# PythonerJOJO/GenPose2

Hardware: AMD Instinct MI355X
Metric: pose candidates/sec (B objs x K cands x T denoise steps) (higher is better)
Workload: dtype f32 (pose_encoder.2 / head-1 GEMMs: f16x3 -- three f16 planes per fp32 operand, six MFMA products, products to 2^-33, fp32 accumulation; encoder SA levels 1-3: split-f16, per-level error vs float64 within exact fp32 MFMA's: tests/test_gpu_precision.py); 1 GPU; config4: B=256 objects/GPU, N=1024 pts, K=50 candidates, T=500 PC steps, ScoreNet+EnergyNet+ranking/aggregation (encoder + sampler per step); global_batch=256, seq_len=500, parallelism=dp1 (object shards), encoder_pipelined=False, energy_encoder=beside the score encoder

## Files before the change

### genpose2_amd/csrc/gp_encoder.hip

```cpp
#include <algorithm>

#include "gp_common.h"
#include "gp_fps.h"
#include "gp_head.h"

int gp_launch_fps_chain(const float* xyz, int b, int nlev, const int* n, const int* m, int* const* idx,
                        float* const* nxyz, hipStream_t st);
int gp_launch_ball_query2(int b, int n, int m, float ra, float rb, int nsa, int nsb, const float* new_xyz,
                          const float* xyz, int* idxa, int* idxb, hipStream_t st);

struct SAArgs {
    int n_prev, c_prev, m, ns, cols;
    const float* xyz_prev;
    const float* feat_prev;
    const float* cent;
    const int* nbr;
    int nlayers;
    const float* w[3];
    const float* bias[3];
    int kg[3];
    int nt[3];
    float* out;
    int c_out_total, out_off;
    int buf1_off;
// ... 501 lines not shown
    f32x4 acc[2 * NC][CT];
#pragma unroll
    for (int t = 0; t < 2 * NC; ++t)
#pragma unroll
        for (int ct = 0; ct < CT; ++ct) acc[t][ct] = f32x4{0.f, 0.f, 0.f, 0.f};
    stream_hk_step<KC1, 0, D, 2 * NC, CT, D>(W, T, X, lane, voff, ring, acc);
    __syncthreads();
    SPLIT_MARK(a, 6);
    stream_hk_step<KC1, D, KC1 + D, 2 * NC, CT, D>(W, T, X, lane, voff, ring, acc);
    const int span = a.ns >> 4;
#pragma unroll
    for (int t = 0; t < 2 * NC; ++t) {
        const f32x4 bias = ld4(a.bias[1] + 16 * T[t] + 4 * q);
        f32x4 v[CT];
#pragma unroll
        for (int ct = 0; ct < CT; ++ct) v[ct] = relu4(acc[t][ct] * exp2i(e1[ct] - 14 - a.ew[1]) + bias);
#pragma unroll
        for (int ct = 0; ct < CT; ++ct) {
            if (span == 2) {
                if (ct & 1) continue;
                v[ct] = vmax4(v[ct], v[ct + 1]);
            }
            const float r = row16_max_scatter4(v[ct], n);
            const int mi = (col0 + ct * 16) / a.ns;
            if ((n & 3) == 0 && mi < a.m) a.out[((size_t)b * a.m + mi) * a.c_out_total + a.out_off + 16 * T[t] + 4 * q + (n >> 2)] = r;
        }
    }
}

template <int CT, int D, int KC0, int OC1, int OC2>
__device__ __forceinline__ void sa_split_body(const SplitArgs& a, char* smem) {
    constexpr int C = 16 * CT, KX = KC0 > OC1 ? KC0 : OC1;
    f16x8* X = reinterpret_cast<f16x8*>(smem);
    float* P = reinterpret_cast<float*>(smem + (size_t)KX * CT * 2048);
    float* pm = P + CT * KC0 * 32;
    int* e0s = reinterpret_cast<int*>(pm + SPLIT_WV * C);
    const int tid = threadIdx.x, lane = tid & 63;
    const int wid = __builtin_amdgcn_readfirstlane(tid >> 6);
    const int b = blockIdx.y, col0 = blockIdx.x * C;
    SPLIT_MARK(a, 0);
    constexpr bool EARLY = KC0 >= 8;
    f32x4 gq[KC0][2];
    const int pnb = wid < CT ? split_gather0_pre(a, b, col0, wid, lane) : 0;
    split_centroid_term<CT, KC0>(a, P, b, col0, tid);
    if (EARLY && wid < CT) split_gather0_load<KC0>(a, b, pnb, lane, gq);
    if constexpr (EARLY) {
        asm volatile("s_waitcnt lgkmcnt(0)\n\ts_barrier" ::: "memory");
    } else {
        __syncthreads();
    }
    SPLIT_MARK(a, 1);
    int e1[CT];
    constexpr int NC1_HI = (OC1 + SPLIT_WV - 1) / SPLIT_WV;
    const int nc1 = wid < OC1 % SPLIT_WV || OC1 % SPLIT_WV == 0 ? NC1_HI : NC1_HI - 1;
    if (nc1 == NC1_HI)
        split_layer1<CT, KC0, NC1_HI, D>(a, X, e0s, pm, reinterpret_cast<const f32x4*>(P), b, col0, wid, lane, OC1, e1, gq, EARLY, pnb);
    else
        split_layer1<CT, KC0, (NC1_HI > 0 ? NC1_HI - 1 : 0), D>(a, X, e0s, pm, reinterpret_cast<const f32x4*>(P), b, col0, wid, lane, OC1, e1, gq, EARLY, pnb);
    static_assert(OC2 % SPLIT_WV == 0, "layer-2 chunks spread evenly over the waves");
    split_layer2<CT, OC1, OC2 / SPLIT_WV, D>(a, X, e1, b, col0, wid, lane, OC2);
    SPLIT_MARK(a, 7);
}

template <int CT, int D, int KC0, int OC1A, int OC2A, int OC1B, int OC2B, int MINB = 1>
__global__ __launch_bounds__(SPLIT_WV * 64) __attribute__((amdgpu_waves_per_eu(2 * MINB))) void sa_split_kernel(SplitArgs a0, SplitArgs a1) {
    extern __shared__ __attribute__((aligned(16))) char smem[];
    if (blockIdx.z == 0) {
        if ((int)blockIdx.x * 16 * CT < a0.cols) sa_split_body<CT, D, KC0, OC1A, OC2A>(a0, smem);
    } else {
        if ((int)blockIdx.x * 16 * CT < a1.cols) sa_split_body<CT, D, KC0, OC1B, OC2B>(a1, smem);
    }
}

#ifndef SPLIT_CT2
#define SPLIT_CT2 4
#endif
#ifndef SPLIT_CT3
#define SPLIT_CT3 6
#endif
#ifndef SPLIT_D2
#define SPLIT_D2 2
#endif
#ifndef SPLIT_D3
#define SPLIT_D3 2
#endif

template <int CT, int KC0, int OC1>
static size_t sa_split_lds() {
    constexpr int KX = KC0 > OC1 ? KC0 : OC1;
    return (size_t)KX * CT * 2048 + sizeof(float) * CT * KC0 * 32 + sizeof(float) * SPLIT_WV * 16 * CT + sizeof(int) * 16 * CT;
}

struct NarrowArgs {
    const float* qin;
    int q_stride, q_off, n_prev;
    const float* w0;
    int kg0, gx;
    const float* w1;
    const float* b1;
    const float* w2;
    const float* b2;
    const int* nbr;
    const float* cent;
    int m, ns, nobj;
    float* out;
    int c_out_total, out_off;
    const float* w1h;
    const float* w2h;
    int ew1, ew2;
};

template <int SPAN, int KG>
struct NarrowGather {
    f32x4 q[SPAN][KG];
    float cx, cy, cz;
};

template <int SPAN>
__device__ __forceinline__ void narrow_nbr(const NarrowArgs& a, int task, int nn, int (&p)[SPAN]) {
#pragma unroll
    for (int ct = 0; ct < SPAN; ++ct) p[ct] = a.nbr[(size_t)task * a.ns + ct * 16 + nn];
}

template <int KG>
__device__ __forceinline__ const f32x4* narrow_centroid_term(const f32x4* sW0x, int q, float cx, float cy, float cz,
                                                             f32x4 (&cw)[KG]) {
#pragma clang fp contract(off)
#pragma unroll
    for (int g = 0; g < KG; ++g) {
        float r[4];
#pragma unroll
        for (int j = 0; j < 4; ++j) {
            const f32x4 wx = sW0x[16 * g + 4 * q + j];
            r[j] = (wx.x * cx + wx.y * cy) + wx.z * cz;
        }
        cw[g] = f32x4{r[0], r[1], r[2], r[3]};
    }
    return cw;
}

template <int SPAN, int KG>
__device__ __forceinline__ void narrow_fetch(const NarrowArgs& a, int task, const int (&p)[SPAN], int q,
                                             NarrowGather<SPAN, KG>& g) {
    const int b = task / a.m;
    const float* cc = a.cent + (size_t)task * 3;
    g.cx = ld1(cc);
    g.cy = ld1(cc + 1);
    g.cz = ld1(cc + 2);
#pragma unroll
    for (int ct = 0; ct < SPAN; ++ct) {
        const float* qrow = a.qin + ((size_t)b * a.n_prev + p[ct]) * a.q_stride + a.q_off + 4 * q;
#pragma unroll
        for (int g2 = 0; g2 < KG; ++g2) g.q[ct][g2] = ld4(qrow + 16 * g2);
    }
}

template <int KG1, int NT1, int NT2, int SPAN>
__device__ __forceinline__ void narrow_branch(const NarrowArgs& a, f32x4* lds) {
    constexpr int KG2 = NT1;
    constexpr int NA1 = NT1 * KG1 * 64, NA2 = NT2 * KG2 * 64;
    f32x4* sA1 = lds;
    f32x4* sA2 = sA1 + NA1;
    f32x4* sW0x = sA2 + NA2;
    float* sB1 = reinterpret_cast<float*>(sW0x + KG1 * 16);
    float* sB2 = sB1 + NT1 * 16;
    const int tid = threadIdx.x;
    for (int i = tid; i < NA1; i += SA_THREADS) sA1[i] = ld4(a.w1 + (size_t)i * 4);
    for (int i = tid; i < NA2; i += SA_THREADS) sA2[i] = ld4(a.w2 + (size_t)i * 4);
    for (int ch = tid; ch < KG1 * 16; ch += SA_THREADS)
        sW0x[ch] = ld4(a.w0 + ((size_t)((ch >> 4) * a.kg0 + a.gx) * 64 + (ch & 15)) * 4);
    for (int i = tid; i < NT1 * 16; i += SA_THREADS) sB1[i] = a.b1[i];
    for (int i = tid; i < NT2 * 16; i += SA_THREADS) sB2[i] = a.b2[i];
    __syncthreads();
    const int lane = tid & 63, q = lane >> 4, nn = lane & 15;
    const int nw = gridDim.x * (SA_THREADS / 64);
    const int total = a.nobj * a.m;
    int task = blockIdx.x * (SA_THREADS / 64) + (tid >> 6);
    if (task >= total) return;
    int pn[SPAN];
    NarrowGather<SPAN, KG1> cur, nxt;
    f32x4 cwv[KG1];
    narrow_nbr<SPAN>(a, task, nn, pn);
    narrow_fetch<SPAN, KG1>(a, task, pn, q, cur);
    if (task + nw < total) narrow_nbr<SPAN>(a, task + nw, nn, pn);
    for (; task < total; task += nw) {
        if (task + nw < total) {
            narrow_fetch<SPAN, KG1>(a, task + nw, pn, q, nxt);
            if (task + 2 * nw < total) narrow_nbr<SPAN>(a, task + 2 * nw, nn, pn);
        }
        const float cx = cur.cx, cy = cur.cy, cz = cur.cz;
        f32x4 rmax[NT2];
#pragma unroll
        for (int t = 0; t < NT2; ++t) rmax[t] = f32x4{NEG_BIG, NEG_BIG, NEG_BIG, NEG_BIG};
        const f32x4* cw = narrow_centroid_term<KG1>(sW0x, q, cx, cy, cz, cwv);
#pragma unroll
        for (int ct = 0; ct < SPAN; ++ct) {
            f32x4 bf[KG1];
#pragma unroll
            for (int g = 0; g < KG1; ++g) {
                float r[4];
#pragma unroll
                for (int j = 0; j < 4; ++j) r[j] = relu1(fsub(cur.q[ct][g][j], cw[g][j]));
                bf[g] = f32x4{r[0], r[1], r[2], r[3]};
            }
            f32x4 acc1[NT1];
#pragma unroll
            for (int t = 0; t < NT1; ++t) acc1[t] = f32x4{0.f, 0.f, 0.f, 0.f};
#pragma unroll
            for (int g = 0; g < KG1; ++g) {
                f32x4 af[NT1];
#pragma unroll
                for (int t = 0; t < NT1; ++t) af[t] = sA1[(t * KG1 + g) * 64 + lane];
#pragma unroll
                for (int j = 0; j < 4; ++j)
#pragma unroll
                    for (int t = 0; t < NT1; ++t) acc1[t] = mfma4(af[t][j], bf[g][j], acc1[t]);
                __builtin_amdgcn_sched_barrier(0);
            }
#pragma unroll
            for (int t = 0; t < NT1; ++t) acc1[t] = relu4(acc1[t] + ld4(&sB1[16 * t + 4 * q]));
            f32x4 acc2[NT2];
#pragma unroll
            for (int t = 0; t < NT2; ++t) acc2[t] = f32x4{0.f, 0.f, 0.f, 0.f};
#pragma unroll
            for (int g = 0; g < KG2; ++g) {
                f32x4 af[NT2];
#pragma unroll
                for (int t = 0; t < NT2; ++t) af[t] = sA2[(t * KG2 + g) * 64 + lane];
#pragma unroll
                for (int j = 0; j < 4; ++j)
#pragma unroll
                    for (int t = 0; t < NT2; ++t) acc2[t] = mfma4(af[t][j], acc1[g][j], acc2[t]);
                __builtin_amdgcn_sched_barrier(0);
            }
#pragma unroll
            for (int t = 0; t < NT2; ++t) rmax[t] = vmax4(rmax[t], acc2[t]);
            __builtin_amdgcn_sched_barrier(0);
        }
        float* o = a.out + (size_t)task * a.c_out_total + a.out_off + 4 * q;
#pragma unroll
        for (int t = 0; t < NT2; ++t) {
            const int j = nn >> 2;
            const float r = relu1(row16_max_scatter4(rmax[t], nn) + sB2[16 * t + 4 * q + j]);
            if ((nn & 3) == 0) o[16 * t + j] = r;
        }
        cur = nxt;
    }
}

template <int KC0, int NT1, int NT2, int SPAN>
__device__ __forceinline__ void narrow_branch_split(const NarrowArgs& a, f32x4* lds) {
    constexpr int KG1 = 2 * KC0, KC1 = NT1 / 2;
    static_assert(NT1 % 2 == 0, "layer-1 tiles pair into 32-deep chunks");
    constexpr int NA1 = NT1 * KC0 * 2 * 64, NA2 = NT2 * KC1 * 2 * 64;
    f16x8* sA1 = reinterpret_cast<f16x8*>(lds);
    f16x8* sA2 = sA1 + NA1;
    f32x4* sW0x = reinterpret_cast<f32x4*>(sA2 + NA2);
    float* sB1 = reinterpret_cast<float*>(sW0x + KG1 * 16);
    float* sB2 = sB1 + NT1 * 16;
    const int tid = threadIdx.x;
    for (int i = tid; i < NA1; i += SA_THREADS) sA1[i] = __builtin_bit_cast(f16x8, ld4(a.w1h + (size_t)i * 4));
    for (int i = tid; i < NA2; i += SA_THREADS) sA2[i] = __builtin_bit_cast(f16x8, ld4(a.w2h + (size_t)i * 4));
    for (int ch = tid; ch < KG1 * 16; ch += SA_THREADS)
        sW0x[ch] = ld4(a.w0 + ((size_t)((ch >> 4) * a.kg0 + a.gx) * 64 + (ch & 15)) * 4);
    for (int i = tid; i < NT1 * 16; i += SA_THREADS) sB1[i] = a.b1[i];
    for (int i = tid; i < NT2 * 16; i += SA_THREADS) sB2[i] = a.b2[i];
    __syncthreads();
    const int lane = tid & 63, q = lane >> 4, nn = lane & 15;
    const int nw = gridDim.x * (SA_THREADS / 64);
    const int total = a.nobj * a.m;
    int task = blockIdx.x * (SA_THREADS / 64) + (tid >> 6);
    if (task >= total) return;
    int pn[SPAN];
    NarrowGather<SPAN, KG1> cur, nxt;
    f32x4 cwv[KG1];
    narrow_nbr<SPAN>(a, task, nn, pn);
    narrow_fetch<SPAN, KG1>(a, task, pn, q, cur);
    if (task + nw < total) narrow_nbr<SPAN>(a, task + nw, nn, pn);
    for (; task < total; task += nw) {
        if (task + nw < total) {
            narrow_fetch<SPAN, KG1>(a, task + nw, pn, q, nxt);
            if (task + 2 * nw < total) narrow_nbr<SPAN>(a, task + 2 * nw, nn, pn);
        }
        const float cx = cur.cx, cy = cur.cy, cz = cur.cz;
        f32x4 rmax[NT2];
#pragma unroll
        for (int t = 0; t < NT2; ++t) rmax[t] = f32x4{NEG_BIG, NEG_BIG, NEG_BIG, NEG_BIG};
        const f32x4* cw = narrow_centroid_term<KG1>(sW0x, q, cx, cy, cz, cwv);
#pragma unroll
        for (int ct = 0; ct < SPAN; ++ct) {
            f32x4 bf[KG1];
            float mx = 0.f;
#pragma unroll
            for (int g = 0; g < KG1; ++g) {
                float r[4];
#pragma unroll
                for (int j = 0; j < 4; ++j) {
                    r[j] = relu1(fsub(cur.q[ct][g][j], cw[g][j]));
                    mx = fmax2(mx, r[j]);
                }
                bf[g] = f32x4{r[0], r[1], r[2], r[3]};
            }
            const int E0 = col_exponent(rows_max(mx));
            f16x8 h0[KC0], l0[KC0];
#pragma unroll
            for (int c = 0; c < KC0; ++c) split_pair(bf[2 * c], bf[2 * c + 1], exp2i(14 - E0), h0[c], l0[c]);
            f32x4 acc1[NT1];
#pragma unroll
            for (int t = 0; t < NT1; ++t) acc1[t] = f32x4{0.f, 0.f, 0.f, 0.f};
#pragma unroll
            for (int c = 0; c < KC0; ++c) {
#pragma unroll
                for (int t = 0; t < NT1; ++t) {
                    const f16x8 ah = sA1[((t * KC0 + c) * 2 + 0) * 64 + lane];
                    const f16x8 al = sA1[((t * KC0 + c) * 2 + 1) * 64 + lane];
                    acc1[t] = mfma_h(al, h0[c], acc1[t]);
                    acc1[t] = mfma_h(ah, l0[c], acc1[t]);
                    acc1[t] = mfma_h(ah, h0[c], acc1[t]);
                }
            }
            const float u0 = exp2i(E0 - 14 - a.ew1);
            float m1 = 0.f;
#pragma unroll
            for (int t = 0; t < NT1; ++t) {
                acc1[t] = relu4(acc1[t] * u0 + ld4(&sB1[16 * t + 4 * q]));
                m1 = fmax2(m1, max4(acc1[t]));
            }
            const int E1 = col_exponent(rows_max(m1));
            f16x8 h1[KC1], l1[KC1];
#pragma unroll
            for (int c = 0; c < KC1; ++c) split_pair(acc1[2 * c], acc1[2 * c + 1], exp2i(14 - E1), h1[c], l1[c]);
            f32x4 acc2[NT2];
#pragma unroll
            for (int t = 0; t < NT2; ++t) acc2[t] = f32x4{0.f, 0.f, 0.f, 0.f};
#pragma unroll
            for (int c = 0; c < KC1; ++c) {
#pragma unroll
                for (int t = 0; t < NT2; ++t) {
                    const f16x8 ah = sA2[((t * KC1 + c) * 2 + 0) * 64 + lane];
                    const f16x8 al = sA2[((t * KC1 + c) * 2 + 1) * 64 + lane];
                    acc2[t] = mfma_h(al, h1[c], acc2[t]);
                    acc2[t] = mfma_h(ah, l1[c], acc2[t]);
                    acc2[t] = mfma_h(ah, h1[c], acc2[t]);
                }
            }
            const float u1 = exp2i(E1 - 14 - a.ew2);
#pragma unroll
            for (int t = 0; t < NT2; ++t) rmax[t] = vmax4(rmax[t], acc2[t] * u1);
            __builtin_amdgcn_sched_barrier(0);
        }
        float* o = a.out + (size_t)task * a.c_out_total + a.out_off + 4 * q;
#pragma unroll
        for (int t = 0; t < NT2; ++t) {
            const int j = nn >> 2;
            const float r = relu1(row16_max_scatter4(rmax[t], nn) + sB2[16 * t + 4 * q + j]);
            if ((nn & 3) == 0) o[16 * t + j] = r;
        }
        cur = nxt;
    }
}

struct FpsSide {
    int nlev;
    int n[2], m[2], nb[2], jbits[2];
    const float* in;
    int* idx[2];
    float* nxyz[2];
    int nobj;
};

static size_t fps_side_lds(const FpsSide& f) {
    return f.nlev ? FPS_RED_BYTES + sizeof(float) * 3 * ((size_t)f.n[0] + f.m[0]) + sizeof(int) * (size_t)f.m[0] : 0;
}

__device__ __forceinline__ void fps_side(const FpsSide& f, char* smem) {
    const int b = blockIdx.x;
    if (b >= f.nobj) return;
    void* s_red = smem;
    float* cur = reinterpret_cast<float*>(smem + FPS_RED_BYTES);
    float* nxt = cur + 3 * f.n[0];
    int* s_idx = reinterpret_cast<int*>(nxt + 3 * f.m[0]);
    const float* src = f.in + (size_t)b * f.n[0] * 3;
    for (int i = threadIdx.x; i < 3 * f.n[0]; i += FPS_THREADS) cur[i] = src[i];
    __syncthreads();
    for (int l = 0; l < f.nlev; ++l) {
        if (f.n[l] <= FPS_THREADS)
            fps_run<1>(cur, f.n[l], f.m[l], f.nb[l], f.jbits[l], s_red, s_idx, nxt);
        else if (f.n[l] <= 2 * FPS_THREADS)
            fps_run<2>(cur, f.n[l], f.m[l], f.nb[l], f.jbits[l], s_red, s_idx, nxt);
        else
            fps_run<4>(cur, f.n[l], f.m[l], f.nb[l], f.jbits[l], s_red, s_idx, nxt);
        __syncthreads();
        int* gi = f.idx[l] + (size_t)b * f.m[l];
        float* gx = f.nxyz[l] + (size_t)b * f.m[l] * 3;
        for (int i = threadIdx.x; i < f.m[l]; i += FPS_THREADS) gi[i] = s_idx[i];
        for (int i = threadIdx.x; i < 3 * f.m[l]; i += FPS_THREADS) gx[i] = nxt[i];
        __syncthreads();
        float* t = cur;
        cur = nxt;
        nxt = t;
    }
}

template <int KG1a, int NT1a, int NT2a, int SPANa, int KG1b, int NT1b, int NT2b, int SPANb>
__global__ __launch_bounds__(SA_THREADS) void sa_narrow_kernel(NarrowArgs a0, NarrowArgs a1, FpsSide f) {
    extern __shared__ __attribute__((aligned(16))) f32x4 lds[];
    if (blockIdx.y == 0)
        fps_side(f, reinterpret_cast<char*>(lds));
    else if (blockIdx.y == 1)
        narrow_branch<KG1a, NT1a, NT2a, SPANa>(a0, lds);
    else
        narrow_branch<KG1b, NT1b, NT2b, SPANb>(a1, lds);
}

template <int KC0a, int NT1a, int NT2a, int SPANa, int KC0b, int NT1b, int NT2b, int SPANb>
__global__ __launch_bounds__(SA_THREADS) void sa_narrow_split_kernel(NarrowArgs a0, NarrowArgs a1, FpsSide f) {
    extern __shared__ __attribute__((aligned(16))) f32x4 lds[];
    if (blockIdx.y == 0)
        fps_side(f, reinterpret_cast<char*>(lds));
    else if (blockIdx.y == 1)
        narrow_branch_split<KC0a, NT1a, NT2a, SPANa>(a0, lds);
    else
        narrow_branch_split<KC0b, NT1b, NT2b, SPANb>(a1, lds);
}

template <int KG1a, int NT1a, int NT2a, int SPANa, int KC0b, int NT1b, int NT2b, int SPANb>
__global__ __launch_bounds__(SA_THREADS) void sa_narrow_mixed_kernel(NarrowArgs a0, NarrowArgs a1, FpsSide f) {
    extern __shared__ __attribute__((aligned(16))) f32x4 lds[];
#ifdef NARROW_PROBE
    if (blockIdx.y != (NARROW_PROBE - 1)) return;
#endif
    if (blockIdx.y == 0)
        fps_side(f, reinterpret_cast<char*>(lds));
// ... 956 lines not shown
```

### genpose2_amd/csrc/gp_head.h

```cpp
#pragma once
#include <type_traits>

#include "gp_common.h"

constexpr int HT = 256;
constexpr int HID = 256;
constexpr int KG_HID = HID / 16;
#ifndef PC_WV1
#define PC_WV1 8
#endif
#ifndef EVAL_WV
#define EVAL_WV 8
#endif
#ifndef PC_D2
#define PC_D2 3
#endif
#ifndef HEAD_PREFETCH
#define HEAD_PREFETCH 2
#endif


#ifndef PC_MARK
#define PC_MARK(k) ((void)trace_slot)
#endif
// ... 229 lines not shown
        }
    }
    if constexpr (!GRAD) __syncthreads();
    PC_MARK(6);
}

#ifndef GRAD_D
#define GRAD_D 4
#endif

template <int WV>
__device__ __forceinline__ void head_backward(const gp_head_grad_weights& gw, const HeadSmem<1, WV>& sm, GradSmem& gs,
                                              int trace_slot = 0) {
    constexpr int TPW = 16 / WV;
    constexpr int KPW = KG_HID / WV;
    constexpr int D = GRAD_D;
    static_assert(KPW * WV == KG_HID && WV * 64 <= KG_HID * 64, "the partial tiles fit g2");
    const int tid = tid_x();
    const int lane = tid & 63;
    const int wid = __builtin_amdgcn_readfirstlane(tid >> 6);
    const int voff = lane * 16;
    const __amdgpu_buffer_rsrc_t WH = make_rsrc(gw.h1p_wt, 3 * HID * HID * 4);
    const __amdgpu_buffer_rsrc_t W2 = make_rsrc(gw.pe2_wt, HID * HID * 4);
    const __amdgpu_buffer_rsrc_t W0 = make_rsrc(gw.pe0_wt, 16 * HID * 4);
    int T2[TPW];
#pragma unroll
    for (int t = 0; t < TPW; ++t) T2[t] = wid * TPW + t;
    f32x4 ring[D + 1][TPW];
    f32x4 acc[TPW][1];
#pragma unroll
    for (int t = 0; t < TPW; ++t) acc[t][0] = f32x4{0.f, 0.f, 0.f, 0.f};
    stream_step<0, D, TPW, 1, 3 * KG_HID, D>(WH, T2, gs.gh, lane, voff, ring, acc);
    __syncthreads();
    PC_MARK(13);
    stream_step<D, 3 * KG_HID + D, TPW, 1, 3 * KG_HID, D>(WH, T2, gs.gh, lane, voff, ring, acc);
#pragma unroll
    for (int t = 0; t < TPW; ++t) {
        gs.g2[T2[t] * 64 + lane] = mask4(acc[t][0], sm.act2[T2[t] * 64 + lane]);
        acc[t][0] = f32x4{0.f, 0.f, 0.f, 0.f};
    }
    f32x4* g1 = gs.gh;
    stream_step<0, D, TPW, 1, KG_HID, D>(W2, T2, gs.g2, lane, voff, ring, acc);
    __syncthreads();
    PC_MARK(14);
    stream_step<D, KG_HID + D, TPW, 1, KG_HID, D>(W2, T2, gs.g2, lane, voff, ring, acc);
#pragma unroll
    for (int t = 0; t < TPW; ++t) g1[T2[t] * 64 + lane] = mask4(acc[t][0], sm.act1[T2[t] * 64 + lane]);
    const int T0[1] = {wid};
    f32x4 ring0[KPW + 1][1];
    f32x4 acc0[1][1] = {{f32x4{0.f, 0.f, 0.f, 0.f}}};
    stream_step<0, KPW, 1, 1, KPW, KPW>(W0, T0, g1, lane, voff, ring0, acc0);
    __syncthreads();
    PC_MARK(15);
    stream_step<KPW, 2 * KPW, 1, 1, KPW, KPW>(W0, T0, g1 + wid * KPW * 64, lane, voff, ring0, acc0);
    gs.g2[wid * 64 + lane] = acc0[0][0];
    __syncthreads();
}

template <int WV>
__device__ __forceinline__ float pose_grad(const GradSmem& gs, int c, int o) {
    float acc = 0.f;
#pragma unroll
    for (int w = 0; w < WV; ++w) acc += gs.g2[w * 64 + 16 * (o >> 2) + c][o & 3];
    return acc;
}

typedef _Float16 f16x8 __attribute__((ext_vector_type(8)));
constexpr int KC_HID = HID / 32;

__device__ __forceinline__ f32x4 mfma_h(f16x8 a, f16x8 b, f32x4 c) {
    return __builtin_amdgcn_mfma_f32_16x16x32_f16(a, b, c, 0, 0, 0);
}
__device__ __forceinline__ float exp2i(int e) {
    e = e < -126 ? -126 : (e > 127 ? 127 : e);
    return __uint_as_float((uint32_t)(e + 127) << 23);
}
__device__ __forceinline__ int ilog2f(float v) { return (int)((__float_as_uint(v) >> 23) & 0xff) - 127; }
__device__ __forceinline__ float rows_max(float v) {
    const auto a = __builtin_amdgcn_permlane16_swap(__float_as_uint(v), __float_as_uint(v), false, false);
    v = fmaxf(__uint_as_float(a[0]), __uint_as_float(a[1]));
    const auto b = __builtin_amdgcn_permlane32_swap(__float_as_uint(v), __float_as_uint(v), false, false);
    return fmaxf(__uint_as_float(b[0]), __uint_as_float(b[1]));
}
__device__ __forceinline__ void split_pair(f32x4 u, f32x4 v, float s, f16x8& hi, f16x8& lo) {
#pragma clang fp contract(off)
    const float x[8] = {u.x * s, u.y * s, u.z * s, u.w * s, v.x * s, v.y * s, v.z * s, v.w * s};
#pragma unroll
    for (int j = 0; j < 8; ++j) {
        const _Float16 h = (_Float16)x[j];
        hi[j] = h;
        lo[j] = (_Float16)(x[j] - (float)h);
    }
}

template <int KC, int G, int GEND, int TT, int NT, int D>
__device__ __forceinline__ void stream_hk_step(__amdgpu_buffer_rsrc_t W, const int (&T)[TT], const f16x8* __restrict__ B,
                                               int lane, int voff, f16x8 (&ring)[D + 1][TT][2], f32x4 (&acc)[TT][NT]) {
    if constexpr (G < GEND) {
        if constexpr (G < KC) {
#pragma unroll
            for (int t = 0; t < TT; ++t)
#pragma unroll
                for (int p = 0; p < 2; ++p)
                    ring[G % (D + 1)][t][p] =
                        __builtin_bit_cast(f16x8, ldbuf4(W, voff, ((T[t] * KC + G) * 2 + p) * 1024));
        }
        __builtin_amdgcn_sched_barrier(0);
        if constexpr (G >= D && NT > 4) {
            constexpr int GG = G - D, S = GG % (D + 1);
#pragma unroll
            for (int ct = 0; ct < NT; ++ct) {
                const f16x8 bh = B[((GG * NT + ct) * 2 + 0) * 64 + lane];
                const f16x8 bl = B[((GG * NT + ct) * 2 + 1) * 64 + lane];
#pragma unroll
                for (int t = 0; t < TT; ++t) acc[t][ct] = mfma_h(ring[S][t][1], bh, acc[t][ct]);
#pragma unroll
                for (int t = 0; t < TT; ++t) acc[t][ct] = mfma_h(ring[S][t][0], bl, acc[t][ct]);
#pragma unroll
                for (int t = 0; t < TT; ++t) acc[t][ct] = mfma_h(ring[S][t][0], bh, acc[t][ct]);
            }
        } else if constexpr (G >= D) {
            constexpr int GG = G - D, S = GG % (D + 1);
            f16x8 bh[NT], bl[NT];
#pragma unroll
            for (int ct = 0; ct < NT; ++ct) {
                bh[ct] = B[((GG * NT + ct) * 2 + 0) * 64 + lane];
                bl[ct] = B[((GG * NT + ct) * 2 + 1) * 64 + lane];
            }
#pragma unroll
            for (int t = 0; t < TT; ++t)
#pragma unroll
                for (int ct = 0; ct < NT; ++ct) acc[t][ct] = mfma_h(ring[S][t][1], bh[ct], acc[t][ct]);
#pragma unroll
            for (int t = 0; t < TT; ++t)
#pragma unroll
                for (int ct = 0; ct < NT; ++ct) acc[t][ct] = mfma_h(ring[S][t][0], bl[ct], acc[t][ct]);
#pragma unroll
            for (int t = 0; t < TT; ++t)
#pragma unroll
                for (int ct = 0; ct < NT; ++ct) acc[t][ct] = mfma_h(ring[S][t][0], bh[ct], acc[t][ct]);
        }
        stream_hk_step<KC, G + 1, GEND, TT, NT, D>(W, T, B, lane, voff, ring, acc);
    }
}


constexpr int HSPLIT_WV = 8;
struct SplitScalars {
    float A0, B0, A2, B2;
    int ew2, ewh;
    f32x4 pe0a[4], pe0b[4];
};
template <int PL, int WV = HSPLIT_WV>
__device__ __forceinline__ SplitScalars load_split_scalars(const gp_head_weights& w) {
    static_assert(WV == 4 || WV == 8, "the split trunk runs 4- or 8-wave workgroups");
    if constexpr (PL == 0) {
        return SplitScalars{};
    } else {
        const f32x4 a = ld4(w.hsc), b = ld4(w.hsc + 4);
        SplitScalars r{a.x, a.y, a.z, a.w, (int)b.x, (int)b.y, {}, {}};
        const int tid = tid_x();
        const int lane = tid & 63, q = lane >> 4;
        const int wid = __builtin_amdgcn_readfirstlane(tid >> 6);
#pragma unroll
        for (int t = 0; t < 16 / WV; ++t) {
            const int T = wid * (16 / WV) + t;
            r.pe0a[t] = ld4(w.pe0_w + ((size_t)T * 64 + lane) * 4);
            r.pe0b[t] = ld4(w.pe0_b + 16 * T + 4 * q);
        }
        return r;
    }
}

__device__ __forceinline__ float rows_sum_scatter4(float a, float b, float c, float d) {
    const auto ab = __builtin_amdgcn_permlane16_swap(__float_as_uint(a), __float_as_uint(b), false, false);
    const auto cd = __builtin_amdgcn_permlane16_swap(__float_as_uint(c), __float_as_uint(d), false, false);
    const float s = __uint_as_float(ab[0]) + __uint_as_float(ab[1]);
    const float t = __uint_as_float(cd[0]) + __uint_as_float(cd[1]);
    const auto st = __builtin_amdgcn_permlane32_swap(__float_as_uint(s), __float_as_uint(t), false, false);
    return __uint_as_float(st[0]) + __uint_as_float(st[1]);
}

struct ColScales {
    float s1, s2, u2, uh, sh;
};
__device__ __forceinline__ ColScales split_col_scales(float m0, const SplitScalars& hs) {
    const float b1 = fmaxf(__builtin_fmaf(hs.A0, m0, hs.B0) * 1.0009765625f, 1e-18f);
    const float b2 = fmaxf(__builtin_fmaf(hs.A2, b1, hs.B2) * 1.0009765625f, 1e-18f);
    const int e1 = ilog2f(b1), e2 = ilog2f(b2);
    return ColScales{exp2i(14 - e1), exp2i(14 - e2), exp2i(e1 - 14 - hs.ew2), exp2i(e2 - 14 - hs.ewh),
                     exp2i(14 - e2 + hs.ewh)};
}
__device__ __forceinline__ float xin_row_absmax(f32x4 b) {
    return rows_max(fmaxf(fmaxf(fabsf(b.x), fabsf(b.y)), fmaxf(fabsf(b.z), fabsf(b.w))));
}

#ifndef X3_D2
#define X3_D2 2
#endif
#ifndef X3_DH
#define X3_DH 1
#endif
constexpr int X3P = 3;

constexpr int X3Q = 4;
typedef int i32x8 __attribute__((ext_vector_type(8)));
typedef unsigned u32x2 __attribute__((ext_vector_type(2)));
constexpr int Q8_EXP_HI = -7, Q8_EXP_MID = 4, Q8_EXP_LO = 16;
template <int PL>
constexpr int act_f16_planes() { return PL == X3Q ? 2 : X3P; }
template <int PL, int NT>
__device__ __forceinline__ constexpr int act_plane(int chunk, int ct, int p) {
    return ((chunk * NT + ct) * act_f16_planes<PL>() + p) * 64;
}
template <int NT>
__device__ __forceinline__ constexpr int act_q8(int group, int ct, int k, int h) {
    return KC_HID * NT * 2 * 64 + (((group * NT + ct) * 3 + k) * 2 + h) * 64;
}
template <int K>
__device__ __forceinline__ f32x4 mfma_q8(f16x8 a0, f16x8 a1, f16x8 b0, f16x8 b1, f32x4 c) {
    using u4 = __attribute__((ext_vector_type(4))) int;
    const u4 x0 = __builtin_bit_cast(u4, a0), x1 = __builtin_bit_cast(u4, a1);
    const u4 y0 = __builtin_bit_cast(u4, b0), y1 = __builtin_bit_cast(u4, b1);
    const i32x8 a = {x0[0], x0[1], x0[2], x0[3], x1[0], x1[1], x1[2], x1[3]};
    const i32x8 b = {y0[0], y0[1], y0[2], y0[3], y1[0], y1[1], y1[2], y1[3]};
    constexpr int ea = K == 0 ? Q8_EXP_HI : (K == 1 ? Q8_EXP_MID : Q8_EXP_LO);
    constexpr int eb = K == 0 ? Q8_EXP_LO : (K == 1 ? Q8_EXP_MID : Q8_EXP_HI);
    return __builtin_amdgcn_mfma_scale_f32_16x16x128_f8f6f4(a, b, c, 0, 0, 0, 127 - ea, 0, 127 - eb);
}
typedef _Float16 f16x2 __attribute__((ext_vector_type(2)));
typedef float f32x2 __attribute__((ext_vector_type(2)));
typedef short i16x2 __attribute__((ext_vector_type(2)));
template <int E, bool VIA_F32 = false>
__device__ __forceinline__ u32x2 q8_of(f16x8 p) {
    if constexpr (VIA_F32) {
        const float s = exp2i(E);
        int lo = 0, hi = 0;
        lo = __builtin_amdgcn_cvt_pk_fp8_f32((float)p[0] * s, (float)p[1] * s, lo, false);
        lo = __builtin_amdgcn_cvt_pk_fp8_f32((float)p[2] * s, (float)p[3] * s, lo, true);
        hi = __builtin_amdgcn_cvt_pk_fp8_f32((float)p[4] * s, (float)p[5] * s, hi, false);
        hi = __builtin_amdgcn_cvt_pk_fp8_f32((float)p[6] * s, (float)p[7] * s, hi, true);
        return u32x2{(unsigned)lo, (unsigned)hi};
    } else {
        const float s = exp2i(-E);
        i16x2 lo, hi;
        asm("" : "=v"(lo) : "v"(f16x2{p[0], p[1]}));
        asm("" : "=v"(hi) : "v"(f16x2{p[4], p[5]}));
        lo = __builtin_amdgcn_cvt_scalef32_pk_fp8_f16(lo, f16x2{p[0], p[1]}, s, false);
        lo = __builtin_amdgcn_cvt_scalef32_pk_fp8_f16(lo, f16x2{p[2], p[3]}, s, true);
        hi = __builtin_amdgcn_cvt_scalef32_pk_fp8_f16(hi, f16x2{p[4], p[5]}, s, false);
        hi = __builtin_amdgcn_cvt_scalef32_pk_fp8_f16(hi, f16x2{p[6], p[7]}, s, true);
        return u32x2{__builtin_bit_cast(unsigned, lo), __builtin_bit_cast(unsigned, hi)};
    }
}
template <int PL>
struct ActPlanes {
    f16x8 h[act_f16_planes<PL>()];
    u32x2 q[PL == X3Q ? 3 : 1];
};

template <int HI>
__device__ __forceinline__ float sub_f16(float x, f16x2 h) {
    float r;
    if constexpr (HI)
        asm("v_fma_mix_f32 %0, %1, -1.0, %2 op_sel:[1,0,0] op_sel_hi:[1,0,0]" : "=v"(r) : "v"(h), "v"(x));
    else
        asm("v_fma_mix_f32 %0, %1, -1.0, %2 op_sel_hi:[1,0,0]" : "=v"(r) : "v"(h), "v"(x));
    return r;
}
__device__ __forceinline__ f16x2 sub_f16_pk(f32x2 x, f16x2 h) {
    f16x2 d;
    asm("v_fma_mixlo_f16 %0, %1, -1.0, %2 op_sel_hi:[1,0,0]" : "=v"(d) : "v"(h), "v"(x[0]));
    asm("v_fma_mixhi_f16 %0, %1, -1.0, %2 op_sel:[1,0,0] op_sel_hi:[1,0,0]" : "+v"(d) : "v"(h), "v"(x[1]));
    return d;
}
__device__ __forceinline__ void split3_pair(f32x4 u, f32x4 v, float s, f16x8 (&p)[X3P]) {
#pragma clang fp contract(off)
    const float x[8] = {u.x * s, u.y * s, u.z * s, u.w * s, v.x * s, v.y * s, v.z * s, v.w * s};
    f16x2 h[4], m[4], l[4];
#pragma unroll
    for (int j = 0; j < 4; ++j) {
        h[j] = __builtin_convertvector(f32x2{x[2 * j], x[2 * j + 1]}, f16x2);
        const f32x2 r = {sub_f16<0>(x[2 * j], h[j]), sub_f16<1>(x[2 * j + 1], h[j])};
        m[j] = __builtin_convertvector(r, f16x2);
        l[j] = sub_f16_pk(r, m[j]);
    }
    p[0] = __builtin_shufflevector(__builtin_shufflevector(h[0], h[1], 0, 1, 2, 3),
                                   __builtin_shufflevector(h[2], h[3], 0, 1, 2, 3), 0, 1, 2, 3, 4, 5, 6, 7);
    p[1] = __builtin_shufflevector(__builtin_shufflevector(m[0], m[1], 0, 1, 2, 3),
                                   __builtin_shufflevector(m[2], m[3], 0, 1, 2, 3), 0, 1, 2, 3, 4, 5, 6, 7);
    p[2] = __builtin_shufflevector(__builtin_shufflevector(l[0], l[1], 0, 1, 2, 3),
                                   __builtin_shufflevector(l[2], l[3], 0, 1, 2, 3), 0, 1, 2, 3, 4, 5, 6, 7);
}
template <int PL>
__device__ __forceinline__ void split_act(f32x4 u, f32x4 v, float s, ActPlanes<PL>& a) {
    f16x8 p[X3P];
    split3_pair(u, v, s, p);
    a.h[0] = p[0];
    a.h[1] = p[1];
    if constexpr (PL == X3Q) {
        a.q[0] = q8_of<Q8_EXP_LO>(p[2]);
        a.q[1] = q8_of<Q8_EXP_MID>(p[1]);
        a.q[2] = q8_of<Q8_EXP_HI>(p[0]);
    } else {
        a.h[2] = p[2];
    }
}
template <int PL, int NT>
__device__ __forceinline__ void store_act(f16x8* act, int chunk, int ct, int lane, const ActPlanes<PL>& a) {
#pragma unroll
    for (int p = 0; p < act_f16_planes<PL>(); ++p) act[act_plane<PL, NT>(chunk, ct, p) + lane] = a.h[p];
    if constexpr (PL == X3Q) {
        const int cc = chunk & 3;
#pragma unroll
        for (int k = 0; k < 3; ++k)
            reinterpret_cast<u32x2*>(act + act_q8<NT>(chunk >> 2, ct, k, cc >> 1) + lane)[cc & 1] = a.q[k];
    }
}
template <int PL>
constexpr int ring_planes() { return PL == X3Q ? 4 : X3P; }
template <int PL, int NT>
__device__ __forceinline__ void load_b_planes(const f16x8* __restrict__ B, int GG, int ct, int lane,
                                              f16x8 (&b)[ring_planes<PL>()]) {
#pragma unroll
    for (int p = 0; p < act_f16_planes<PL>(); ++p) b[p] = B[act_plane<PL, NT>(GG, ct, p) + lane];
    if constexpr (PL == X3Q) {
        if ((GG & 3) < 3) {
            b[2] = B[act_q8<NT>(GG >> 2, ct, GG & 3, 0) + lane];
            b[3] = B[act_q8<NT>(GG >> 2, ct, GG & 3, 1) + lane];
        }
    }
}
template <int PL, int KQ>
__device__ __forceinline__ f32x4 cross_products(const f16x8 (&w)[ring_planes<PL>()], const f16x8 (&b)[ring_planes<PL>()],
                                                f32x4 c) {
    if constexpr (PL != X3Q) {
        c = mfma_h(w[2], b[0], c);
        c = mfma_h(w[0], b[2], c);
        c = mfma_h(w[1], b[1], c);
    }
    c = mfma_h(w[1], b[0], c);
    c = mfma_h(w[0], b[1], c);
    if constexpr (PL == X3Q && KQ < 3) c = mfma_q8<KQ < 3 ? KQ : 0>(w[2], w[3], b[2], b[3], c);
    return c;
}
template <int PL, int G, int GEND, int TT, int NT, int D>
__device__ __forceinline__ void stream_x3_rec(__amdgpu_buffer_rsrc_t W, __amdgpu_buffer_rsrc_t WQ, const int (&T)[TT],
                                              const f16x8* __restrict__ B, int lane, int voff,
                                              f16x8 (&ring)[D + 1][TT][ring_planes<PL>()], f32x4 (&acc)[TT][NT],
                                              f32x4 (&cor)[TT][NT], f16x8 (&bc)[ring_planes<PL>()]) {
    constexpr int RP = ring_planes<PL>();
    if constexpr (G < GEND) {
        if constexpr (G < KC_HID) {
#pragma unroll
            for (int t = 0; t < TT; ++t) {
#pragma unroll
                for (int p = 0; p < act_f16_planes<PL>(); ++p)
                    ring[G % (D + 1)][t][p] =
                        __builtin_bit_cast(f16x8, ldbuf4(W, voff, ((T[t] * KC_HID + G) * X3P + p) * 1024));
                if constexpr (PL == X3Q && (G & 3) < 3) {
#pragma unroll
                    for (int h = 0; h < 2; ++h)
                        ring[G % (D + 1)][t][2 + h] = __builtin_bit_cast(
                            f16x8, ldbuf4(WQ, voff, (((T[t] * (KC_HID / 4) + G / 4) * 3 + (G & 3)) * 2 + h) * 1024));
                }
            }
        }
        __builtin_amdgcn_sched_barrier(0);
        if constexpr (G >= D) {
            constexpr int GG = G - D, S = GG % (D + 1), KQ = GG & 3;
            if constexpr (GG == 0) load_b_planes<PL, NT>(B, 0, 0, lane, bc);
#pragma unroll
            for (int ct = 0; ct < NT; ++ct) {
                f16x8 bn[RP];
                const int ng = ct + 1 < NT ? GG : GG + 1, nc = ct + 1 < NT ? ct + 1 : 0;
                if (ct + 1 < NT || GG + 1 < KC_HID) load_b_planes<PL, NT>(B, ng, nc, lane, bn);
// ... 451 lines not shown
```

Baseline: 265.2 million pose-candidate-steps/s.

## Software-pipeline LDS weight fragments in narrow SA branch and head streaming

```diff
diff --git a/genpose2_amd/csrc/gp_encoder.hip b/genpose2_amd/csrc/gp_encoder.hip
--- a/genpose2_amd/csrc/gp_encoder.hip
+++ b/genpose2_amd/csrc/gp_encoder.hip
@@ -607,7 +607,7 @@
 #define SPLIT_D2 2
 #endif
 #ifndef SPLIT_D3
-#define SPLIT_D3 2
+#define SPLIT_D3 1
 #endif
 
 template <int CT, int KC0, int OC1>
@@ -773,10 +773,37 @@
     }
 }
 
+constexpr int NARROW_PF = 2;
+template <int KC0, int NT1, int NT2>
+__device__ __forceinline__ void narrow_frag(const f16x8* sA1, const f16x8* sA2, int r, int lane, f16x8 (&f)[2]) {
+    constexpr int KC1 = NT1 / 2, S1 = KC0 * NT1;
+    const f16x8* src = r < S1 ? sA1 + ((r % NT1) * KC0 + r / NT1) * 2 * 64
+                              : sA2 + (((r - S1) % NT2) * KC1 + (r - S1) / NT2) * 2 * 64;
+    f[0] = src[lane];
+    f[1] = src[64 + lane];
+}
+template <int KC0, int NT1, int NT2, int SPAN, int NT>
+__device__ __forceinline__ void narrow_step(const f16x8* sA1, const f16x8* sA2, int r, int lane,
+                                            f16x8 (&fq)[NARROW_PF + 1][2], const f16x8 (&h)[SPAN], const f16x8 (&l)[SPAN],
+                                            f32x4 (&acc)[SPAN][NT], int t) {
+    constexpr int ST = KC0 * NT1 + NT1 / 2 * NT2;
+    narrow_frag<KC0, NT1, NT2>(sA1, sA2, (r + NARROW_PF) % ST, lane, fq[(r + NARROW_PF) % (NARROW_PF + 1)]);
+    __builtin_amdgcn_sched_barrier(0);
+    const f16x8 ah = fq[r % (NARROW_PF + 1)][0], al = fq[r % (NARROW_PF + 1)][1];
+#pragma unroll
+    for (int ct = 0; ct < SPAN; ++ct) {
+        acc[ct][t] = mfma_h(al, h[ct], acc[ct][t]);
+        acc[ct][t] = mfma_h(ah, l[ct], acc[ct][t]);
+        acc[ct][t] = mfma_h(ah, h[ct], acc[ct][t]);
+    }
+}
+
 template <int KC0, int NT1, int NT2, int SPAN>
 __device__ __forceinline__ void narrow_branch_split(const NarrowArgs& a, f32x4* lds) {
     constexpr int KG1 = 2 * KC0, KC1 = NT1 / 2;
     static_assert(NT1 % 2 == 0, "layer-1 tiles pair into 32-deep chunks");
+    constexpr int S1 = KC0 * NT1, ST = S1 + KC1 * NT2;
+    static_assert(ST % (NARROW_PF + 1) == 0, "the fragment slots line up from task to task");
     constexpr int NA1 = NT1 * KC0 * 2 * 64, NA2 = NT2 * KC1 * 2 * 64;
     f16x8* sA1 = reinterpret_cast<f16x8*>(lds);
     f16x8* sA2 = sA1 + NA1;
@@ -802,6 +829,9 @@
     narrow_nbr<SPAN>(a, task, nn, pn);
     narrow_fetch<SPAN, KG1>(a, task, pn, q, cur);
     if (task + nw < total) narrow_nbr<SPAN>(a, task + nw, nn, pn);
+    f16x8 fq[NARROW_PF + 1][2];
+#pragma unroll
+    for (int r = 0; r < NARROW_PF; ++r) narrow_frag<KC0, NT1, NT2>(sA1, sA2, r, lane, fq[r]);
     for (; task < total; task += nw) {
         if (task + nw < total) {
             narrow_fetch<SPAN, KG1>(a, task + nw, pn, q, nxt);
@@ -812,6 +842,8 @@
 #pragma unroll
         for (int t = 0; t < NT2; ++t) rmax[t] = f32x4{NEG_BIG, NEG_BIG, NEG_BIG, NEG_BIG};
         const f32x4* cw = narrow_centroid_term<KG1>(sW0x, q, cx, cy, cz, cwv);
+        int E0[SPAN];
+        f16x8 h0[KC0][SPAN], l0[KC0][SPAN];
 #pragma unroll
         for (int ct = 0; ct < SPAN; ++ct) {
             f32x4 bf[KG1];
@@ -826,54 +858,54 @@
                 }
                 bf[g] = f32x4{r[0], r[1], r[2], r[3]};
             }
-            const int E0 = col_exponent(rows_max(mx));
-            f16x8 h0[KC0], l0[KC0];
-#pragma unroll
-            for (int c = 0; c < KC0; ++c) split_pair(bf[2 * c], bf[2 * c + 1], exp2i(14 - E0), h0[c], l0[c]);
-            f32x4 acc1[NT1];
-#pragma unroll
-            for (int t = 0; t < NT1; ++t) acc1[t] = f32x4{0.f, 0.f, 0.f, 0.f};
-#pragma unroll
-            for (int c = 0; c < KC0; ++c) {
-#pragma unroll
-                for (int t = 0; t < NT1; ++t) {
-                    const f16x8 ah = sA1[((t * KC0 + c) * 2 + 0) * 64 + lane];
-                    const f16x8 al = sA1[((t * KC0 + c) * 2 + 1) * 64 + lane];
-                    acc1[t] = mfma_h(al, h0[c], acc1[t]);
-                    acc1[t] = mfma_h(ah, l0[c], acc1[t]);
-                    acc1[t] = mfma_h(ah, h0[c], acc1[t]);
-                }
-            }
-            const float u0 = exp2i(E0 - 14 - a.ew1);
+            E0[ct] = col_exponent(rows_max(mx));
+#pragma unroll
+            for (int c = 0; c < KC0; ++c)
+                split_pair(bf[2 * c], bf[2 * c + 1], exp2i(14 - E0[ct]), h0[c][ct], l0[c][ct]);
+        }
+        f32x4 acc1[SPAN][NT1];
+#pragma unroll
+        for (int ct = 0; ct < SPAN; ++ct)
+#pragma unroll
+            for (int t = 0; t < NT1; ++t) acc1[ct][t] = f32x4{0.f, 0.f, 0.f, 0.f};
+#pragma unroll
+        for (int c = 0; c < KC0; ++c)
+#pragma unroll
+            for (int t = 0; t < NT1; ++t)
+                narrow_step<KC0, NT1, NT2, SPAN, NT1>(sA1, sA2, c * NT1 + t, lane, fq, h0[c], l0[c], acc1, t);
+        int E1[SPAN];
+        f16x8 h1[KC1][SPAN], l1[KC1][SPAN];
+#pragma unroll
+        for (int ct = 0; ct < SPAN; ++ct) {
+            const float u0 = exp2i(E0[ct] - 14 - a.ew1);
             float m1 = 0.f;
 #pragma unroll
             for (int t = 0; t < NT1; ++t) {
-                acc1[t] = relu4(acc1[t] * u0 + ld4(&sB1[16 * t + 4 * q]));
-                m1 = fmax2(m1, max4(acc1[t]));
-            }
-            const int E1 = col_exponent(rows_max(m1));
-            f16x8 h1[KC1], l1[KC1];
-#pragma unroll
-            for (int c = 0; c < KC1; ++c) split_pair(acc1[2 * c], acc1[2 * c + 1], exp2i(14 - E1), h1[c], l1[c]);
-            f32x4 acc2[NT2];
-#pragma unroll
-            for (int t = 0; t < NT2; ++t) acc2[t] = f32x4{0.f, 0.f, 0.f, 0.f};
-#pragma unroll
-            for (int c = 0; c < KC1; ++c) {
-#pragma unroll
-                for (int t = 0; t < NT2; ++t) {
-                    const f16x8 ah = sA2[((t * KC1 + c) * 2 + 0) * 64 + lane];
-                    const f16x8 al = sA2[((t * KC1 + c) * 2 + 1) * 64 + lane];
-                    acc2[t] = mfma_h(al, h1[c], acc2[t]);
-                    acc2[t] = mfma_h(ah, l1[c], acc2[t]);
-                    acc2[t] = mfma_h(ah, h1[c], acc2[t]);
-                }
-            }
-            const float u1 = exp2i(E1 - 14 - a.ew2);
-#pragma unroll
-            for (int t = 0; t < NT2; ++t) rmax[t] = vmax4(rmax[t], acc2[t] * u1);
-            __builtin_amdgcn_sched_barrier(0);
-        }
+                acc1[ct][t] = relu4(acc1[ct][t] * u0 + ld4(&sB1[16 * t + 4 * q]));
+                m1 = fmax2(m1, max4(acc1[ct][t]));
+            }
+            E1[ct] = col_exponent(rows_max(m1));
+#pragma unroll
+            for (int c = 0; c < KC1; ++c)
+                split_pair(acc1[ct][2 * c], acc1[ct][2 * c + 1], exp2i(14 - E1[ct]), h1[c][ct], l1[c][ct]);
+        }
+        f32x4 acc2[SPAN][NT2];
+#pragma unroll
+        for (int ct = 0; ct < SPAN; ++ct)
+#pragma unroll
+            for (int t = 0; t < NT2; ++t) acc2[ct][t] = f32x4{0.f, 0.f, 0.f, 0.f};
+#pragma unroll
+        for (int c = 0; c < KC1; ++c)
+#pragma unroll
+            for (int t = 0; t < NT2; ++t)
+                narrow_step<KC0, NT1, NT2, SPAN, NT2>(sA1, sA2, S1 + c * NT2 + t, lane, fq, h1[c], l1[c], acc2, t);
+#pragma unroll
+        for (int ct = 0; ct < SPAN; ++ct) {
+            const float u1 = exp2i(E1[ct] - 14 - a.ew2);
+#pragma unroll
+            for (int t = 0; t < NT2; ++t) rmax[t] = vmax4(rmax[t], acc2[ct][t] * u1);
+        }
+        __builtin_amdgcn_sched_barrier(0);
         float* o = a.out + (size_t)task * a.c_out_total + a.out_off + 4 * q;
 #pragma unroll
         for (int t = 0; t < NT2; ++t) {
diff --git a/genpose2_amd/csrc/gp_head.h b/genpose2_amd/csrc/gp_head.h
--- a/genpose2_amd/csrc/gp_head.h
+++ b/genpose2_amd/csrc/gp_head.h
@@ -335,20 +335,11 @@
     const auto b = __builtin_amdgcn_permlane32_swap(__float_as_uint(v), __float_as_uint(v), false, false);
     return fmaxf(__uint_as_float(b[0]), __uint_as_float(b[1]));
 }
-__device__ __forceinline__ void split_pair(f32x4 u, f32x4 v, float s, f16x8& hi, f16x8& lo) {
-#pragma clang fp contract(off)
-    const float x[8] = {u.x * s, u.y * s, u.z * s, u.w * s, v.x * s, v.y * s, v.z * s, v.w * s};
-#pragma unroll
-    for (int j = 0; j < 8; ++j) {
-        const _Float16 h = (_Float16)x[j];
-        hi[j] = h;
-        lo[j] = (_Float16)(x[j] - (float)h);
-    }
-}
-
-template <int KC, int G, int GEND, int TT, int NT, int D>
-__device__ __forceinline__ void stream_hk_step(__amdgpu_buffer_rsrc_t W, const int (&T)[TT], const f16x8* __restrict__ B,
-                                               int lane, int voff, f16x8 (&ring)[D + 1][TT][2], f32x4 (&acc)[TT][NT]) {
+
+template <int KC, int G, int GEND, int TT, int NT, int D, int PF>
+__device__ __forceinline__ void stream_hk_rec(__amdgpu_buffer_rsrc_t W, const int (&T)[TT], const f16x8* __restrict__ B,
+                                              int lane, int voff, f16x8 (&ring)[D + 1][TT][2], f32x4 (&acc)[TT][NT],
+                                              f16x8 (&bq)[PF + 1][2]) {
     if constexpr (G < GEND) {
         if constexpr (G < KC) {
 #pragma unroll
@@ -359,44 +350,41 @@
                         __builtin_bit_cast(f16x8, ldbuf4(W, voff, ((T[t] * KC + G) * 2 + p) * 1024));
         }
         __builtin_amdgcn_sched_barrier(0);
-        if constexpr (G >= D && NT > 4) {
-            constexpr int GG = G - D, S = GG % (D + 1);
+        if constexpr (G >= D) {
+            constexpr int GG = G - D, S = GG % (D + 1), NJ = KC * NT;
+            if constexpr (GG == 0) {
+#pragma unroll
+                for (int j = 0; j < PF && j < NJ; ++j)
+#pragma unroll
+                    for (int p = 0; p < 2; ++p) bq[j % (PF + 1)][p] = B[(j * 2 + p) * 64 + lane];
+            }
 #pragma unroll
             for (int ct = 0; ct < NT; ++ct) {
-                const f16x8 bh = B[((GG * NT + ct) * 2 + 0) * 64 + lane];
-                const f16x8 bl = B[((GG * NT + ct) * 2 + 1) * 64 + lane];
+                const int j = GG * NT + ct, jn = j + PF;
+                if (jn < NJ) {
+#pragma unroll
+                    for (int p = 0; p < 2; ++p) bq[jn % (PF + 1)][p] = B[(jn * 2 + p) * 64 + lane];
+                }
+                __builtin_amdgcn_sched_barrier(0);
+                const f16x8 bh = bq[j % (PF + 1)][0], bl = bq[j % (PF + 1)][1];
 #pragma unroll
                 for (int t = 0; t < TT; ++t) acc[t][ct] = mfma_h(ring[S][t][1], bh, acc[t][ct]);
 #pragma unroll
                 for (int t = 0; t < TT; ++t) acc[t][ct] = mfma_h(ring[S][t][0], bl, acc[t][ct]);
 #pragma unroll
                 for (int t = 0; t < TT; ++t) acc[t][ct] = mfma_h(ring[S][t][0], bh, acc[t][ct]);
-            }
-        } else if constexpr (G >= D) {
-            constexpr int GG = G - D, S = GG % (D + 1);
-            f16x8 bh[NT], bl[NT];
-#pragma unroll
-            for (int ct = 0; ct < NT; ++ct) {
-                bh[ct] = B[((GG * NT + ct) * 2 + 0) * 64 + lane];
-                bl[ct] = B[((GG * NT + ct) * 2 + 1) * 64 + lane];
-            }
-#pragma unroll
-            for (int t = 0; t < TT; ++t)
-#pragma unroll
-                for (int ct = 0; ct < NT; ++ct) acc[t][ct] = mfma_h(ring[S][t][1], bh[ct], acc[t][ct]);
-#pragma unroll
-            for (int t = 0; t < TT; ++t)
-#pragma unroll
-                for (int ct = 0; ct < NT; ++ct) acc[t][ct] = mfma_h(ring[S][t][0], bl[ct], acc[t][ct]);
-#pragma unroll
-            for (int t = 0; t < TT; ++t)
-#pragma unroll
-                for (int ct = 0; ct < NT; ++ct) acc[t][ct] = mfma_h(ring[S][t][0], bh[ct], acc[t][ct]);
-        }
-        stream_hk_step<KC, G + 1, GEND, TT, NT, D>(W, T, B, lane, voff, ring, acc);
-    }
-}
-
+                __builtin_amdgcn_sched_barrier(0);
+            }
+        }
+        stream_hk_rec<KC, G + 1, GEND, TT, NT, D, PF>(W, T, B, lane, voff, ring, acc, bq);
+    }
+}
+template <int KC, int G, int GEND, int TT, int NT, int D, int PF = (NT > 4 ? 1 : 2)>
+__device__ __forceinline__ void stream_hk_step(__amdgpu_buffer_rsrc_t W, const int (&T)[TT], const f16x8* __restrict__ B,
+                                               int lane, int voff, f16x8 (&ring)[D + 1][TT][2], f32x4 (&acc)[TT][NT]) {
+    f16x8 bq[PF + 1][2];
+    stream_hk_rec<KC, G, GEND, TT, NT, D, PF>(W, T, B, lane, voff, ring, acc, bq);
+}
 
 constexpr int HSPLIT_WV = 8;
 struct SplitScalars {
@@ -545,6 +533,21 @@
     p[2] = __builtin_shufflevector(__builtin_shufflevector(l[0], l[1], 0, 1, 2, 3),
                                    __builtin_shufflevector(l[2], l[3], 0, 1, 2, 3), 0, 1, 2, 3, 4, 5, 6, 7);
 }
+__device__ __forceinline__ void split_pair(f32x4 u, f32x4 v, float s, f16x8& hi, f16x8& lo) {
+#pragma clang fp contract(off)
+    const float x[8] = {u.x * s, u.y * s, u.z * s, u.w * s, v.x * s, v.y * s, v.z * s, v.w * s};
+    f16x2 h[4], l[4];
+#pragma unroll
+    for (int j = 0; j < 4; ++j) {
+        const f32x2 xx = {x[2 * j], x[2 * j + 1]};
+        h[j] = __builtin_convertvector(xx, f16x2);
+        l[j] = sub_f16_pk(xx, h[j]);
+    }
+    hi = __builtin_shufflevector(__builtin_shufflevector(h[0], h[1], 0, 1, 2, 3),
+                                 __builtin_shufflevector(h[2], h[3], 0, 1, 2, 3), 0, 1, 2, 3, 4, 5, 6, 7);
+    lo = __builtin_shufflevector(__builtin_shufflevector(l[0], l[1], 0, 1, 2, 3),
+                                 __builtin_shufflevector(l[2], l[3], 0, 1, 2, 3), 0, 1, 2, 3, 4, 5, 6, 7);
+}
 template <int PL>
 __device__ __forceinline__ void split_act(f32x4 u, f32x4 v, float s, ActPlanes<PL>& a) {
     f16x8 p[X3P];
```

Measured after the change: 267.0 million pose-candidate-steps/s (median of 6 runs). Within noise of the previous version (+0.7%).
